# OpenBMB/VisRAG

Measured on AMD Instinct MI355X. Metric: page-images embedded/sec (VisRAG-Ret encode, 448x448, bf16 MFMA) + queries/sec@top-10 over 100k-page index, higher is better.
Workload: dtype bf16; 1 GPU; VisRAG-Ret (SigLIP-so400m 26 blk + resampler + MiniCPM-2B 40 layers) bf16 encode batch=32 page images 448x448 per GPU; index 100000 rows x 2304 sharded 1 way(s), 1000 queries top-10; batch_per_gpu=32, global_batch=32, parallelism=dp1 (pages sharded, no data-path collective)

## Files before the change

visrag_amd/csrc/gemm256w.hip:

```cpp
#include <type_traits>

#include "gemm_core.h"
#include "gemm_epilogue.h"
#include "gemm256w_acc.h"

namespace vr {

bool gemm256w_fits(const GemmArgs& a, int bn);

namespace {

constexpr int W_STAGE = 2 * G256_TILE_BYTES;
constexpr unsigned W_OOB = 0x80000000u;

}

constexpr int W_STAGING = 4096;
constexpr int W_WARM_DUMP = 256;
constexpr int W_SMEM_BYTES = 2 * W_STAGE + 4 * W_STAGING + 4 * W_WARM_DUMP;

constexpr bool warm_shares_tile(size_t bytes, unsigned total) {
    unsigned at = 0;
    for (unsigned w = 0; w < total; ++w)
        for (unsigned v = 0; v < WARM_WAVES; ++v) {
            const WarmShare s = warm_share(bytes, w, total, v);
            if (s.first != at || s.end < s.first) return false;
            at = s.end;
        }
    return at == warm_lines(bytes) && (size_t)at * WARM_LINE >= bytes && (bytes == 0 || (size_t)(at - 1) * WARM_LINE < bytes);
}
static_assert(warm_shares_tile(0, 1) && warm_shares_tile(0, 243), "no lines");
static_assert(warm_shares_tile(1, 1) && warm_shares_tile(WARM_LINE, 4) && warm_shares_tile(WARM_LINE + 1, 4), "1 and 2 lines");
static_assert(warm_shares_tile(63 * WARM_LINE, 1) && warm_shares_tile(64 * WARM_LINE, 1) && warm_shares_tile(65 * WARM_LINE, 1), "63 / 64 / 65 lines, one workgroup");
static_assert(warm_shares_tile(63 * WARM_LINE, 4) && warm_shares_tile(64 * WARM_LINE, 4) && warm_shares_tile(65 * WARM_LINE - 3, 4), "63 / 64 / 65 lines, four");
static_assert(warm_shares_tile(100 * WARM_LINE, 243) && warm_shares_tile(5 * WARM_LINE, 405), "a region of fewer lines than the grid has waves");
static_assert(warm_shares_tile((size_t)2304 * 2304 * 2, 243), "W_o (10.6 MB) over the decoder's q|k|v grid");
static_assert(warm_shares_tile((size_t)2304 * 5760 * 2, 405), "W_down (26.5 MB) over the decoder's gate|up grid");
static_assert(warm_shares_tile(WARM_MAX_BYTES - 1, 1021), "the largest region");
static_assert(warm_cut((1u << 24) - 1, 65534, 65535) == (unsigned)(((1ull << 24) - 1) * 65534 / 65535) && warm_cut(65534, 65534, 65535) == 65533 &&
              warm_cut((1u << 24) - 1, 65535, 65535) == (1u << 24) - 1, "the largest grid of the 32-bit form");
static_assert(warm_part(0, warm_lines(WARM_MAX_BYTES - 1), 65536, 65537).end == warm_lines(WARM_MAX_BYTES - 1) &&
              warm_cut(1u << 24, 70001, 70003) == (unsigned)((1ull << 24) * 70001 / 70003) && warm_cut(82944, 100, 243) == 82944ull * 100 / 243, "both forms of the cut");
#if VR_WARM_LINE == 128
static_assert(warm_instructions(warm_share((size_t)2304 * 2304 * 2, 0, 243, 0)) == 2 &&
              warm_instructions(warm_share((size_t)2304 * 5760 * 2, 404, 405, 3)) == 2, "two requests per wave in the decoder");
#endif

#define W_KERNEL_TEMPLATE template <int EPI, bool PLAIN, int NJ>
#define W_KERNEL_NAME gemm256w_bf16_kernel
#include "gemm256w_kernel.h"
#undef W_KERNEL_TEMPLATE
#undef W_KERNEL_NAME

template <int EPI, bool PLAIN, int NJ>
static hipError_t launch_wp(GemmArgs a, hipStream_t s) {
    constexpr int BN = 32 * NJ;
    const int tn = (a.N + BN - 1) / BN, tm = (a.M + G256_BM - 1) / G256_BM;
    if (a.raster_gm <= 0) a.raster_gm = tm <= 16 ? tm : 4;
    if (!gemm256w_fits(a, BN)) return hipErrorInvalidValue;
    if (gemm_args_refused(a, EPI, NJ == 6 ? GEMM_VARIANT_192W : GEMM_VARIANT_256W)) return hipErrorInvalidValue;
    int total = tn * tm;
    if (a.ksplit > 1) total *= a.ksplit;
    auto k = gemm256w_bf16_kernel<EPI, PLAIN, NJ>;
    static unsigned long long attr = 0;
    set_max_dynamic_lds((const void*)k, W_SMEM_BYTES, attr);
    hipLaunchKernelGGL(k, dim3(total), dim3(256), W_SMEM_BYTES, s, a);
    return hipGetLastError();
}

template <int EPI>
static hipError_t launch_w(const GemmArgs& a, hipStream_t s) {
    if constexpr (EPI == EPI_BF16 || EPI == EPI_GELU || EPI == EPI_SWIGLU || EPI == EPI_ROPE) {
        const bool rb_ok = !a.rowbias || (EPI == EPI_BF16 && a.rowbias_period > 0 && a.rowbias_period % G256_BM == 0 && a.rowbias_cols % 64 == 0 && a.rowbias_cols <= a.rowbias_ld &&
                                          (size_t)a.rowbias_period * a.rowbias_ld * 4 < (1ull << 32));
        if (!a.rowmap && rb_ok && (a.N & 7) == 0 && (a.ldo & 7) == 0) return launch_wp<EPI, true, 8>(a, s);
    }
    return launch_wp<EPI, false, 8>(a, s);
}

bool gemm256w_fits(const GemmArgs& a, int bn) {
    const size_t tm = (a.M + G256_BM - 1) / G256_BM, tn = (a.N + bn - 1) / bn;
    return tm * G256_BM * (size_t)a.lda * 2 < (1ull << 31) && tn * bn * (size_t)a.ldw * 2 < (1ull << 31) &&
           (size_t)G256_BM * (size_t)a.ldo * 4 < (1ull << 31) && (!a.rowbias || (size_t)G256_BM * (size_t)a.rowbias_ld * 4 < (1ull << 31));
}

hipError_t launch_gemm256w(const GemmArgs& a, int epi, hipStream_t s) {
    switch (epi) {
        case EPI_BF16: return launch_w<EPI_BF16>(a, s);
        case EPI_GELU: return launch_w<EPI_GELU>(a, s);
        case EPI_F32: return launch_w<EPI_F32>(a, s);
        case EPI_RESID: return launch_w<EPI_RESID>(a, s);
        case EPI_SWIGLU: return launch_w<EPI_SWIGLU>(a, s);
        case EPI_ROPE: return launch_w<EPI_ROPE>(a, s);
        default: return hipErrorInvalidValue;
    }
}

hipError_t launch_gemm192w(const GemmArgs& a, int epi, hipStream_t s) {
    if (a.N % 192) return hipErrorInvalidValue;
    if (epi == EPI_RESID && a.ksplit <= 1) return launch_wp<EPI_RESID, false, 6>(a, s);
    if (epi == EPI_F32) return launch_wp<EPI_F32, false, 6>(a, s);
    return hipErrorInvalidValue;
}

}
```

visrag_amd/csrc/gemm256w_kernel.h:

```cpp
W_KERNEL_TEMPLATE
__global__ __launch_bounds__(256) __attribute__((amdgpu_waves_per_eu(1, 1))) void W_KERNEL_NAME(GemmArgs p) {
    static_assert(NJ == 8 || (NJ == 6 && !PLAIN), "wave tile 128 x 128 or 128 x 96");
    constexpr int BN = 32 * NJ;
    constexpr int NS = 8 * NJ;
    constexpr int NR = 8 + NJ;
    constexpr int DS = NJ == 8 ? 5 : 4;
    constexpr int SB1 = NS * 5 / 8;
    constexpr int D1 = (NS - 1 - (SB1 + 2)) / DS + 1;
    constexpr int SB2 = NJ;
    constexpr int NF = NJ / 2;
    static_assert(SB2 + 3 + DS * (NR - D1 - 1) < NS && SB2 + 2 + 2 * (NR - 1) < NS && 2 * NR - 2 < SB1, "schedule fits");
    extern __shared__ __attribute__((aligned(16))) char smem[];
#ifdef VR_W_TIMING
    const unsigned long long tm0 = __builtin_amdgcn_s_memrealtime();
    unsigned long long tm1 = 0, tm2 = 0, cy1 = 0, cy2 = 0;
#endif
    const int tiles_n = (p.N + BN - 1) / BN;
    const int tiles_m = (p.M + G256_BM - 1) / G256_BM;
    const int ks = p.ksplit > 1 ? p.ksplit : 1;
    const int total = tiles_m * tiles_n * ks;
    const int Ks = p.K / ks;
    const int nk = Ks / GEMM_BK;

    const int my_first = xcd_remap(blockIdx.x, total);
// ... 31 lines not shown

    typedef const __attribute__((address_space(3))) bf16x8* frag_p;
    frag_p pA[2][2], pW[2][2];
#pragma unroll
    for (int st = 0; st < 2; ++st)
#pragma unroll
        for (int kk = 0; kk < 2; ++kk) {
            const int ch = ((kk * 4 + fq) ^ (fr & 7)) << 4;
            pA[st][kk] = (frag_p)VR_LDS(smem + st * W_STAGE + (wm * 128 + fr) * 128 + ch);
            pW[st][kk] = (frag_p)VR_LDS(smem + st * W_STAGE + G256_TILE_BYTES + (wn * 16 * NJ + fr) * 128 + ch);
            asm volatile("" : "+v"(pA[st][kk]), "+v"(pW[st][kk]));
        }

    bf16x8 a0[8], w0[NJ], a1[8], w1[NJ];
    int m0, n0, split;
    coords(my_first, m0, n0, split);
    unsigned curA = tile_off_a(m0, split), curW = tile_off_w(n0, split);
    unsigned warm_lo = 0, warm_hi = 0;

    {
        const unsigned k1 = nk > 1 ? (unsigned)(GEMM_BK * 2) : W_OOB;
#pragma unroll
        for (int d = 0; d < NR; ++d) dma(0, d, lofA + curA, lofW + curW);
#pragma unroll
        for (int d = 0; d < NR; ++d) dma(1, d, lofA + curA + k1, lofW + curW + k1);
        if constexpr (NJ == 8) {
            if (p.warm && p.warm_bytes) {
                const WarmShare sh = warm_share(p.warm_bytes, (unsigned)my_first, (unsigned)total, (unsigned)wave);
                warm_lo = (unsigned)__builtin_amdgcn_readfirstlane((int)sh.first);
                warm_hi = (unsigned)__builtin_amdgcn_readfirstlane((int)sh.end);
            }
        }
        W_FOR_EACH_ACC(W_ZERO)
        if constexpr (NJ == 8) VR_WAIT_VM_BARRIER(16); else VR_WAIT_VM_BARRIER(14);
#pragma unroll
        for (int j = 0; j < NJ; ++j) w0[j] = pW[0][0][j * 128];
#pragma unroll
        for (int i = 0; i < 8; ++i) a0[i] = pA[0][0][i * 128];
    }
#ifdef VR_W_TIMING
    asm volatile("s_waitcnt lgkmcnt(0)" ::: "memory");
    tm1 = __builtin_amdgcn_s_memrealtime();
    cy1 = __builtin_amdgcn_s_memtime();
#endif

    {
        const unsigned nxtA = W_OOB, nxtW = W_OOB;

        auto step = [&](auto stage_c, int kt) {
            constexpr int S = decltype(stage_c)::value;
            const int k2 = kt + 2;
            const unsigned vA = lofA + (k2 < nk ? curA + (unsigned)k2 * (GEMM_BK * 2) : nxtA + (unsigned)(k2 - nk) * (GEMM_BK * 2));
            const unsigned vW = lofW + (k2 < nk ? curW + (unsigned)k2 * (GEMM_BK * 2) : nxtW + (unsigned)(k2 - nk) * (GEMM_BK * 2));
            __builtin_amdgcn_sched_barrier(0);
            auto aux1 = [&](int sl) {
                if (sl < 2 * NR && (sl & 1) == 0) {
                    const int q = sl >> 1;
                    if (q < NJ) w1[q] = pW[S][1][q * 128];
                    else a1[q - NJ] = pA[S][1][(q - NJ) * 128];
                }
                if (sl == SB1) asm volatile("s_waitcnt lgkmcnt(0)\n\ts_barrier" ::: "memory");
                if (sl >= SB1 + 2 && (sl - (SB1 + 2)) % DS == 0) dma(S, (sl - (SB1 + 2)) / DS, vA, vW);
                __builtin_amdgcn_sched_barrier(0);
            };
            auto aux2 = [&](int sl) {
                if (sl == SB2) { if constexpr (D1 == 5) VR_WAIT_VM_BARRIER(5); else VR_WAIT_VM_BARRIER(4); }
                if (sl >= SB2 + 3 && (sl - (SB2 + 3)) % DS == 0 && D1 + (sl - (SB2 + 3)) / DS < NR)
                    dma(S, D1 + (sl - (SB2 + 3)) / DS, vA, vW);
                if (sl >= SB2 + 2 && sl < SB2 + 2 + 2 * NR && ((sl - SB2) & 1) == 0) {
                    const int q = (sl - (SB2 + 2)) >> 1;
                    if (q < NJ) w0[q] = pW[S ^ 1][0][q * 128];
                    else a0[q - NJ] = pA[S ^ 1][0][(q - NJ) * 128];
                }
                __builtin_amdgcn_sched_barrier(0);
            };
#define W_P1(n, R, C0, C1, C2, C3) \
            if (((n) & 7) < NJ) { W_MFMA(R, C0, C1, C2, C3, w0[(n) & 7], a0[(n) >> 3]); aux1(((n) >> 3) * NJ + ((n) & 7)); }
#define W_P2(n, R, C0, C1, C2, C3) \
            if (((n) & 7) < NJ) { W_MFMA(R, C0, C1, C2, C3, w1[(n) & 7], a1[(n) >> 3]); aux2(((n) >> 3) * NJ + ((n) & 7)); }
            W_FOR_EACH_ACC(W_P1)
            W_FOR_EACH_ACC(W_P2)
#undef W_P1
#undef W_P2
        };

        for (int kt = 0; kt < nk; kt += 2) {
            step(std::integral_constant<int, 0>{}, kt);
            if (kt + 1 >= nk) break;
            step(std::integral_constant<int, 1>{}, kt + 1);
        }
        asm volatile("s_nop 15\n\ts_nop 15" ::: "memory");
#ifdef VR_W_TIMING
        tm2 = __builtin_amdgcn_s_memrealtime();
        cy2 = __builtin_amdgcn_s_memtime();
#endif

        const int mrow0 = m0 + wm * 128, nb0 = n0 + wn * (16 * NJ);
        char* const wl0 = smem + 2 * W_STAGE + wave * W_STAGING;
        bool plain_resid = false;
        if constexpr (EPI == EPI_RESID) plain_resid = !p.rowmap;
        auto uni32 = [](unsigned v) { return (unsigned)__builtin_amdgcn_readfirstlane((int)v); };
        auto uni_ptr = [&](const void* q) {
            const unsigned long long a = (unsigned long long)q;
            return (void*)(((unsigned long long)uni32((unsigned)(a >> 32)) << 32) | uni32((unsigned)a));
        };
        auto warm_requests = [&]() {
            if constexpr (NJ == 8) {
                if (warm_lo < warm_hi) {
                    const unsigned long long wa = (unsigned long long)uni_ptr(p.warm);
                    const auto wrs = __builtin_amdgcn_make_buffer_rsrc((void*)wa, 0, uni32((unsigned)p.warm_bytes), 0x00020000);
                    const unsigned pad = (0u - (unsigned)wa) & 3u;
                    char* const dump = smem + 2 * W_STAGE + 4 * W_STAGING + wave * W_WARM_DUMP;
                    auto request = [&](unsigned l) {
                        const unsigned line = l + (unsigned)lane;
                        __builtin_amdgcn_raw_ptr_buffer_load_lds(wrs, VR_LDS(dump), 4, line < warm_hi ? line * WARM_LINE + pad : W_OOB, 0, 0, 0);
                    };
                    __builtin_amdgcn_sched_barrier(0);
                    request(warm_lo);
                    request(warm_lo + 64);
                    __builtin_amdgcn_sched_barrier(0);
#pragma nounroll
                    for (unsigned l = warm_lo + 128; l < warm_hi; l += 64) request(l);
                }
            }
        };
        bool buf_tile = false;
        if constexpr (EPI == EPI_RESID) buf_tile = plain_resid && n0 + BN <= p.N;
        if constexpr (EPI == EPI_F32) buf_tile = !p.rowmap && !p.rowbias && n0 + BN <= p.N;
        if constexpr (EPI == EPI_RESID || EPI == EPI_F32) {
            if (buf_tile) {
                constexpr int MI = 2;
                const float alpha = __builtin_bit_cast(float, uni32(__builtin_bit_cast(unsigned, p.alpha)));
                const unsigned ldb = uni32((unsigned)p.ldo * 4u);
                const unsigned nrec = uni32((unsigned)min(G256_BM, p.M - m0) * ldb);
                float* obase = (float*)p.out + (size_t)m0 * p.ldo;
                if constexpr (EPI == EPI_F32) obase += (size_t)split * p.split_stride;
                const auto ors = __builtin_amdgcn_make_buffer_rsrc(uni_ptr(obase), 0, nrec, 0x00020000);
                const bool with_bias = p.bias && (EPI == EPI_RESID || split == 0);
                const auto brs = __builtin_amdgcn_make_buffer_rsrc(uni_ptr(p.bias), 0, uni32(with_bias ? (unsigned)p.N * 4u : 0u), 0x00020000);
                const unsigned voff = (unsigned)(wm * 128 + fr) * ldb + (unsigned)(nb0 + fq * 4) * 4u;
                f32x4 bias[NJ];
#pragma unroll
                for (int j = 0; j < NJ; ++j)
                    bias[j] = __builtin_bit_cast(f32x4, __builtin_amdgcn_raw_buffer_load_b128(brs, (unsigned)(nb0 + fq * 4) * 4u + j * 64, 0, 0));
                if constexpr (EPI == EPI_RESID) {
                    constexpr int RD = NJ == 6 ? 3 : 2;
                    const auto rrs = __builtin_amdgcn_make_buffer_rsrc(uni_ptr(p.resid + (size_t)m0 * p.ldo), 0, nrec, 0x00020000);
                    f32x4 rs[RD + 1][MI][NF];
                    auto load_piece = [&](int q, f32x4 (&dst)[MI][NF]) {
                        const int h = q & 1, sg = q >> 1;
#pragma unroll
                        for (int i = 0; i < MI; ++i)
#pragma unroll
                            for (int j = 0; j < NF; ++j)
                                dst[i][j] = __builtin_bit_cast(f32x4, __builtin_amdgcn_raw_buffer_load_b128(
                                    rrs, voff + (unsigned)((sg * MI + i) * 16) * ldb + (h * NF + j) * 64, 0, 0));
                    };
#pragma unroll
                    for (int q = 0; q < RD; ++q) load_piece(q, rs[q]);
                    warm_requests();
#pragma unroll
                    for (int q = 0; q < 8; ++q) {
                        const int h = q & 1, sg = q >> 1;
                        if (q + RD < 8) load_piece(q + RD, rs[(q + RD) % (RD + 1)]);
                        f32x4 acc[MI][NF];
#define W_RD(n, R, C0, C1, C2, C3) \
                        if (((n) & 7) < NJ && ((n) & 7) / NF == h && ((n) >> 4) == sg) W_READ(acc[((n) >> 3) & 1][((n) & 7) % NF], C0, C1, C2, C3);
                        W_FOR_EACH_ACC(W_RD)
#undef W_RD
#pragma unroll
                        for (int i = 0; i < MI; ++i)
#pragma unroll
                            for (int j = 0; j < NF; ++j) {
                                const f32x4 v = rs[q % (RD + 1)][i][j] + alpha * (acc[i][j] + bias[h * NF + j]);
                                __builtin_amdgcn_raw_buffer_store_b128(__builtin_bit_cast(u32x4, v), ors,
                                                                       voff + (unsigned)((sg * MI + i) * 16) * ldb + (h * NF + j) * 64, 0, 0);
                            }
                        __builtin_amdgcn_sched_barrier(0);
                    }
                } else {
                    warm_requests();
#pragma unroll
                    for (int q = 0; q < 8; ++q) {
                        const int h = q & 1, sg = q >> 1;
                        f32x4 acc[MI][NF];
#define W_RD(n, R, C0, C1, C2, C3) \
                        if (((n) & 7) < NJ && ((n) & 7) / NF == h && ((n) >> 4) == sg) W_READ(acc[((n) >> 3) & 1][((n) & 7) % NF], C0, C1, C2, C3);
                        W_FOR_EACH_ACC(W_RD)
#undef W_RD
#pragma unroll
                        for (int i = 0; i < MI; ++i)
#pragma unroll
                            for (int j = 0; j < NF; ++j)
                                __builtin_amdgcn_raw_buffer_store_b128(__builtin_bit_cast(u32x4, acc[i][j] + bias[h * NF + j]), ors,
                                                                       voff + (unsigned)((sg * MI + i) * 16) * ldb + (h * NF + j) * 64, 0, 0);
                        __builtin_amdgcn_sched_barrier(0);
                    }
                }
            }
        }
        if constexpr (EPI == EPI_RESID) {
            if (plain_resid && !buf_tile) {
                constexpr int MI = 2;
                const float* __restrict__ resid = p.resid;
                float* __restrict__ out = (float*)p.out;
                constexpr int RD = 1;
                f32x4 rs[RD + 1][MI][NF];
                auto load_piece = [&](int q, f32x4 (&dst)[MI][NF]) {
                    const int h = q & 1, sg = q >> 1;
#pragma unroll
                    for (int i = 0; i < MI; ++i) {
                        const size_t ro = (size_t)min(mrow0 + (sg * MI + i) * 16 + fr, p.M - 1) * p.ldo;
#pragma unroll
                        for (int j = 0; j < NF; ++j) {
                            dst[i][j] = *reinterpret_cast<const f32x4*>(resid + ro + min(nb0 + (h * NF + j) * 16 + fq * 4, p.N - 4));
                        }
                    }
                };
#pragma unroll
                for (int q = 0; q < RD; ++q) load_piece(q, rs[q]);
                f32x4 bias[NJ];
#pragma unroll
                for (int j = 0; j < NJ; ++j)
                    bias[j] = p.bias ? *reinterpret_cast<const f32x4*>(p.bias + min(nb0 + j * 16 + fq * 4, p.N - 4)) : f32x4{0.f, 0.f, 0.f, 0.f};
                warm_requests();
#pragma unroll
                for (int q = 0; q < 8; ++q) {
                    const int h = q & 1, sg = q >> 1;
                    if (q + RD < 8) load_piece(q + RD, rs[(q + RD) % (RD + 1)]);
                    f32x4 acc[MI][NF];
#define W_RD(n, R, C0, C1, C2, C3) \
                    if (((n) & 7) < NJ && ((n) & 7) / NF == h && ((n) >> 4) == sg) W_READ(acc[((n) >> 3) & 1][((n) & 7) % NF], C0, C1, C2, C3);
                    W_FOR_EACH_ACC(W_RD)
#undef W_RD
#pragma unroll
                    for (int i = 0; i < MI; ++i) {
                        const int m = mrow0 + (sg * MI + i) * 16 + fr;
#pragma unroll
                        for (int j = 0; j < NF; ++j) {
                            const int n = nb0 + (h * NF + j) * 16 + fq * 4;
                            if (m < p.M && n < p.N)
                                *reinterpret_cast<f32x4*>(out + (size_t)m * p.ldo + n) = rs[q % (RD + 1)][i][j] + p.alpha * (acc[i][j] + bias[h * NF + j]);
                        }
                    }
                    __builtin_amdgcn_sched_barrier(0);
                }
            }
        }
        if (!plain_resid && !buf_tile) {
            const unsigned ldo2 = uni32((unsigned)p.ldo * 2u);
            const auto ors16 = __builtin_amdgcn_make_buffer_rsrc(uni_ptr((const char*)p.out + (size_t)m0 * p.ldo * 2), 0,
                                                                 uni32((unsigned)min(G256_BM, p.M - m0) * ldo2), 0x00020000);
            f32x4 biasw[NJ];
            if constexpr (PLAIN && NF == 4 && EPI != EPI_ROPE) {
                const auto brs = __builtin_amdgcn_make_buffer_rsrc(uni_ptr(p.bias), 0, uni32(p.bias ? (unsigned)p.N * 4u : 0u), 0x00020000);
#pragma unroll
                for (int j = 0; j < NJ; ++j)
                    biasw[j] = __builtin_bit_cast(f32x4, __builtin_amdgcn_raw_buffer_load_b128(brs, (unsigned)(nb0 + fq * 4) * 4u + j * 64, 0, 0));
            }
            const bool rb_on = EPI == EPI_BF16 && PLAIN && p.rowbias != nullptr;
            const auto rbrs = __builtin_amdgcn_make_buffer_rsrc(uni_ptr(p.rowbias), 0,
                                                                uni32(rb_on ? (unsigned)p.rowbias_period * (unsigned)p.rowbias_ld * 4u : 0u), 0x00020000);
            const unsigned rb_row0 = rb_on ? uni32((unsigned)(m0 % p.rowbias_period)) : 0u;
            int posw[8];
#pragma unroll
            for (int t = 0; t < 8; ++t) posw[t] = 0;
            if constexpr (EPI == EPI_ROPE && PLAIN) {
#pragma unroll
                for (int t = 0; t < 8; ++t) posw[t] = p.rope_pos[min(mrow0 + t * 16 + fr, p.M - 1)];
            }
            f32x4 rt[2][2][4];
            auto load_rope = [&](int sg, f32x4 (&d)[2][4]) {
#pragma unroll
                for (int i = 0; i < 2; ++i) {
                    const float* tab = p.rope_table + (size_t)posw[sg * 2 + i] * 64 + fq * 4;
#pragma unroll
                    for (int j = 0; j < 4; ++j) d[i][j] = *reinterpret_cast<const f32x4*>(tab + j * 16);
                }
            };
            if constexpr (EPI == EPI_ROPE && PLAIN) load_rope(0, rt[0]);
            (void)ors16; (void)ldo2; (void)biasw; (void)rbrs; (void)rb_row0; (void)posw; (void)rt;
            warm_requests();
#pragma unroll
            for (int q = 0; q < 8; ++q) {
                constexpr int MI = 2;
                const int h = q & 1, sg = q >> 1;
                f32x4 acc[MI][NF];
#define W_RD(n, R, C0, C1, C2, C3) \
                if (((n) & 7) < NJ && ((n) & 7) / NF == h && ((n) >> 4) == sg) W_READ(acc[((n) >> 3) & 1][((n) & 7) % NF], C0, C1, C2, C3);
                W_FOR_EACH_ACC(W_RD)
#undef W_RD
                const int mr = mrow0 + sg * 32, nb = nb0 + h * (16 * NF);
                bool done = false;
                if constexpr (EPI == EPI_F32) {
                    if (!p.rowmap && !p.rowbias) {
                        float* __restrict__ out = (float*)p.out + (size_t)split * p.split_stride;
                        const float* bp = split == 0 ? p.bias : nullptr;
                        f32x4 bias[NF];
#pragma unroll
                        for (int j = 0; j < NF; ++j)
                            bias[j] = bp ? *reinterpret_cast<const f32x4*>(bp + min(nb + j * 16 + fq * 4, p.N - 4)) : f32x4{0.f, 0.f, 0.f, 0.f};
#pragma unroll
                        for (int i = 0; i < MI; ++i) {
                            const int m = mr + i * 16 + fr;
#pragma unroll
                            for (int j = 0; j < NF; ++j) {
                                const int n = nb + j * 16 + fq * 4;
                                if (m < p.M && n < p.N) *reinterpret_cast<f32x4*>(out + (size_t)m * p.ldo + n) = acc[i][j] + bias[j];
                            }
                        }
                        done = true;
                    } else if (ks > 1) {
                        GemmArgs ps = p;
                        ps.out = (float*)p.out + (size_t)split * p.split_stride;
                        if (split > 0) ps.bias = nullptr;
#pragma unroll
                        for (int i = 0; i < MI; ++i) gemm_epilogue_row<EPI_F32, NF>(acc[i], ps, mr + i * 16 + fr, nb, fq);
                        done = true;
                    }
                }
                if constexpr (EPI == EPI_RESID) {
#pragma unroll
                    for (int i = 0; i < MI; ++i) gemm_epilogue_row<EPI_RESID, NF>(acc[i], p, mr + i * 16 + fr, nb, fq);
                    done = true;
                }
                if constexpr (NF == 4 && (EPI == EPI_BF16 || EPI == EPI_GELU || EPI == EPI_SWIGLU || EPI == EPI_ROPE)) {
                    if constexpr (PLAIN) {
                        f32x4 b4[4];
#pragma unroll
                        for (int j = 0; j < 4; ++j) b4[j] = EPI == EPI_ROPE ? f32x4{0.f, 0.f, 0.f, 0.f} : biasw[h * NF + j];
                        if constexpr (EPI == EPI_ROPE) { if (h == 0 && sg + 1 < 4) load_rope(sg + 1, rt[(sg + 1) & 1]); }
                        gemm_epilogue_tile_lds_plain_buf<EPI, MI>(acc, b4, p, ors16, (unsigned)(wm * 128 + sg * 32) * ldo2, ldo2, rt[sg & 1], nb, lane, wl0,
                                                                  rbrs, (rb_row0 + (unsigned)(wm * 128 + sg * 32)) * (unsigned)p.rowbias_ld * 4u);
                        done = true;
                    } else if ((p.N & 7) == 0 && (p.ldo & 7) == 0) {
                        gemm_epilogue_tile_lds<EPI, MI>(acc, p, mr, nb, lane, wl0);
                        done = true;
                    }
                }
                if constexpr (!PLAIN) {
                    if (!done) {
#pragma unroll
                        for (int i = 0; i < MI; ++i) gemm_epilogue_row<EPI, NF>(acc[i], p, mr + i * 16 + fr, nb, fq);
                    }
                }
                if (!PLAIN || (q & 1)) __builtin_amdgcn_sched_barrier(0);
            }
        }
    }
#ifdef VR_W_TIMING
    if (threadIdx.x == 0 && p.rope_table) {
        const unsigned long long tm3 = __builtin_amdgcn_s_memrealtime();
        asm volatile("s_waitcnt vmcnt(0)" ::: "memory");
        const unsigned long long tm4 = __builtin_amdgcn_s_memrealtime();
        unsigned long long* d = (unsigned long long*)p.rope_table + (size_t)blockIdx.x * 16;
        d[0] = tm0; d[1] = tm1; d[2] = tm2; d[3] = tm3; d[4] = tm4;
        d[5] = __builtin_amdgcn_s_getreg((31 << 11) | 4);
        d[6] = __builtin_amdgcn_s_getreg((31 << 11) | 20);
        d[7] = cy2 - cy1;
    }
#endif
}
```

visrag_amd/csrc/gemm_epilogue.h:

```cpp
#pragma once
#include "common.h"
#include "kernels.h"

namespace vr {

__device__ __forceinline__ float gelu_erf(float x) {
    constexpr float X0 = 4.2426406871192851f;
    const float xc = fminf(fmaxf(x, -X0), X0);
    const float u = xc * xc;
    float p = 1.125353832e-10f;
    p = fmaf(p, u, -1.074373991e-08f);
    p = fmaf(p, u, 4.536592962e-07f);
    p = fmaf(p, u, -1.129243078e-05f);
    p = fmaf(p, u, 1.871812565e-04f);
    p = fmaf(p, u, -2.218800626e-03f);
    p = fmaf(p, u, 1.963623831e-02f);
    p = fmaf(p, u, -1.326938473e-01f);
    p = fmaf(p, u, 7.978062550e-01f);
    const float e = xc * p;
    const float hx = 0.5f * x;
    return fmaf(hx, e, hx);
}
__device__ __forceinline__ f32x4 gelu_erf4(f32x4 x) {
    constexpr float X0 = 4.2426406871192851f;
// ... 196 lines not shown
    if constexpr (EPI == EPI_SWIGLU) {
#pragma unroll
        for (int it = 0; it < MI; ++it) {
            const int row = it * 16 + (lane >> 2), c = lane & 3;
            const u32x4 d = *reinterpret_cast<const u32x4*>(wl + row * 128 + ((c ^ (row & 3)) << 4));
            const int m = mrow0 + row, n = nb / 2 + c * 8;
            if (m < p.M && 2 * n < p.N) {
                const int orow = p.rowmap ? p.rowmap[m] : m;
                if (orow >= 0) *reinterpret_cast<u32x4*>(out + (size_t)orow * p.ldo + n) = d;
            }
        }
    } else {
#pragma unroll
        for (int it = 0; it < MI * 2; ++it) {
            const int row = it * 8 + (lane >> 3), c = lane & 7;
            const u32x4 d = *reinterpret_cast<const u32x4*>(wl + row * 128 + ((c ^ (row & 7)) << 4));
            const int m = mrow0 + row, n = nb + c * 8;
            if (m < p.M && n < p.N) {
                const int orow = p.rowmap ? p.rowmap[m] : m;
                if (orow >= 0) *reinterpret_cast<u32x4*>(out + (size_t)orow * p.ldo + n) = d;
            }
        }
    }
}

template <int EPI, int MI>
__device__ __forceinline__ void gemm_epilogue_tile_lds_plain(f32x4 (&acc)[MI][4], const GemmArgs& p, int mrow0, int nb,
                                                             int lane, char* wl_generic) {
    typedef __attribute__((address_space(3))) char* lds_p;
    const lds_p wl = (lds_p)VR_LDS(wl_generic);
    const int fr = lane & 15, fq = lane >> 4;
    if constexpr (EPI == EPI_SWIGLU) {
        f32x4 bias[4];
#pragma unroll
        for (int j = 0; j < 4; ++j) bias[j] = f32x4{0.f, 0.f, 0.f, 0.f};
        if (p.bias) {
#pragma unroll
            for (int j = 0; j < 4; ++j) bias[j] = *reinterpret_cast<const f32x4*>(p.bias + min(nb + j * 16 + fq * 4, p.N - 4));
        }
#pragma unroll
        for (int i = 0; i < MI; ++i) {
            const int row = i * 16 + fr;
#pragma unroll
            for (int jj = 0; jj < 2; ++jj) {
                const f32x4 g = acc[i][2 * jj] + bias[2 * jj], u = acc[i][2 * jj + 1] + bias[2 * jj + 1];
                bf16x4 o;
#pragma unroll
                for (int r = 0; r < 4; ++r) o[r] = f2bf(silu(g[r]) * u[r]);
                const int c = jj * 2 + (fq >> 1);
                *reinterpret_cast<__attribute__((address_space(3))) bf16x4*>(wl + row * 128 + ((c ^ (row & 3)) << 4) + (fq & 1) * 8) = o;
            }
        }
    } else {
        f32x4 bias[4];
#pragma unroll
        for (int j = 0; j < 4; ++j) bias[j] = f32x4{0.f, 0.f, 0.f, 0.f};
        if constexpr (EPI == EPI_BF16 || EPI == EPI_GELU) {
            if (p.bias) {
#pragma unroll
                for (int j = 0; j < 4; ++j) bias[j] = *reinterpret_cast<const f32x4*>(p.bias + min(nb + j * 16 + fq * 4, p.N - 4));
            }
        }
        if constexpr (EPI == EPI_ROPE) {
            if (nb < p.rope_cols && nb < p.N) {
                int pos[MI];
#pragma unroll
                for (int i = 0; i < MI; ++i) pos[i] = p.rope_pos[min(mrow0 + i * 16 + fr, p.M - 1)];
#pragma unroll
                for (int c = 0; c < MI; c += 2) {
                    f32x4 cs[2][2], sn[2][2];
#pragma unroll
                    for (int ii = 0; ii < 2; ++ii) {
                        const float* tab = p.rope_table + (size_t)pos[c + ii] * 64;
#pragma unroll
                        for (int j = 0; j < 2; ++j) {
                            cs[ii][j] = *reinterpret_cast<const f32x4*>(tab + j * 16 + fq * 4);
                            sn[ii][j] = *reinterpret_cast<const f32x4*>(tab + 32 + j * 16 + fq * 4);
                        }
                    }
#pragma unroll
                    for (int ii = 0; ii < 2; ++ii)
#pragma unroll
                        for (int j = 0; j < 2; ++j) {
                            const f32x4 x1 = acc[c + ii][j], x2 = acc[c + ii][j + 2];
                            acc[c + ii][j] = x1 * cs[ii][j] - x2 * sn[ii][j];
                            acc[c + ii][j + 2] = x2 * cs[ii][j] + x1 * sn[ii][j];
                        }
                }
            }
        }
        if constexpr (EPI == EPI_BF16) {
            if (nb < p.col_scale_n) {
#pragma unroll
                for (int j = 0; j < 4; ++j) {
                    bias[j] *= p.col_scale;
#pragma unroll
                    for (int i = 0; i < MI; ++i) acc[i][j] *= p.col_scale;
                }
            }
        }
#pragma unroll
        for (int i = 0; i < MI; ++i) {
            const int row = i * 16 + fr;
#pragma unroll
            for (int j = 0; j < 4; ++j) {
                f32x4 v = acc[i][j] + bias[j];
                if constexpr (EPI == EPI_GELU) v = gelu_erf4(v);
                const bf16x4 o = __builtin_convertvector(v, bf16x4);
                const int c = j * 2 + (fq >> 1);
                *reinterpret_cast<__attribute__((address_space(3))) bf16x4*>(wl + row * 128 + ((c ^ (row & 7)) << 4) + (fq & 1) * 8) = o;
            }
        }
    }
    bf16_t* out = (bf16_t*)p.out;
    if constexpr (EPI == EPI_SWIGLU) {
        u32x4 d[MI];
#pragma unroll
        for (int it = 0; it < MI; ++it) {
            const int row = it * 16 + (lane >> 2), c = lane & 3;
            d[it] = *reinterpret_cast<const __attribute__((address_space(3))) u32x4*>(wl + row * 128 + ((c ^ (row & 3)) << 4));
        }
#pragma unroll
        for (int it = 0; it < MI; ++it) {
            const int row = it * 16 + (lane >> 2), c = lane & 3;
            const int m = mrow0 + row, n = nb / 2 + c * 8;
            if (m < p.M && 2 * n < p.N) *reinterpret_cast<u32x4*>(out + (size_t)m * p.ldo + n) = d[it];
        }
    } else {
        u32x4 d[MI * 2];
#pragma unroll
        for (int it = 0; it < MI * 2; ++it) {
            const int row = it * 8 + (lane >> 3), c = lane & 7;
            d[it] = *reinterpret_cast<const __attribute__((address_space(3))) u32x4*>(wl + row * 128 + ((c ^ (row & 7)) << 4));
        }
#pragma unroll
        for (int it = 0; it < MI * 2; ++it) {
            const int row = it * 8 + (lane >> 3), c = lane & 7;
            const int m = mrow0 + row, n = nb + c * 8;
            if (m < p.M && n < p.N) *reinterpret_cast<u32x4*>(out + (size_t)m * p.ldo + n) = d[it];
        }
    }
}

template <int EPI, int MI>
__device__ __forceinline__ void gemm_epilogue_tile_lds_plain_buf(f32x4 (&acc)[MI][4], f32x4 (&bias)[4], const GemmArgs& p,
                                                                 __amdgpu_buffer_rsrc_t ors, unsigned row_off, unsigned ldo_bytes,
                                                                 const f32x4 (&rope)[MI][4], int nb, int lane, char* wl_generic,
                                                                 __amdgpu_buffer_rsrc_t rbrs, unsigned rb_off) {
    static_assert(EPI == EPI_BF16 || EPI == EPI_GELU || EPI == EPI_SWIGLU || EPI == EPI_ROPE, "bf16 outputs only");
    typedef __attribute__((address_space(3))) char* lds_p;
    const lds_p wl = (lds_p)VR_LDS(wl_generic);
    const int fr = lane & 15, fq = lane >> 4;
    if constexpr (EPI == EPI_SWIGLU) {
#pragma unroll
        for (int i = 0; i < MI; ++i) {
            const int row = i * 16 + fr;
#pragma unroll
            for (int jj = 0; jj < 2; ++jj) {
                const f32x4 g = acc[i][2 * jj] + bias[2 * jj], u = acc[i][2 * jj + 1] + bias[2 * jj + 1];
                bf16x4 o;
#pragma unroll
                for (int r = 0; r < 4; ++r) o[r] = f2bf(silu(g[r]) * u[r]);
                const int c = jj * 2 + (fq >> 1);
                *reinterpret_cast<__attribute__((address_space(3))) bf16x4*>(wl + row * 128 + ((c ^ (row & 3)) << 4) + (fq & 1) * 8) = o;
            }
        }
    } else {
        if constexpr (EPI == EPI_ROPE) {
            if (nb < p.rope_cols && nb < p.N) {
#pragma unroll
                for (int i = 0; i < MI; ++i)
#pragma unroll
                    for (int j = 0; j < 2; ++j) {
                        const f32x4 x1 = acc[i][j], x2 = acc[i][j + 2];
                        acc[i][j] = x1 * rope[i][j] - x2 * rope[i][2 + j];
                        acc[i][j + 2] = x2 * rope[i][j] + x1 * rope[i][2 + j];
                    }
            }
        }
        if constexpr (EPI == EPI_BF16) {
            if (p.rowbias && nb < p.rowbias_cols) {
                f32x4 rb[MI][4];
#pragma unroll
                for (int i = 0; i < MI; ++i)
#pragma unroll
                    for (int j = 0; j < 4; ++j)
                        rb[i][j] = __builtin_bit_cast(f32x4, __builtin_amdgcn_raw_buffer_load_b128(
                            rbrs, rb_off + (unsigned)(i * 16 + fr) * (unsigned)p.rowbias_ld * 4u + (unsigned)(nb + j * 16 + fq * 4) * 4u, 0, 0));
#pragma unroll
                for (int i = 0; i < MI; ++i)
#pragma unroll
                    for (int j = 0; j < 4; ++j) acc[i][j] += rb[i][j];
            }
            if (nb < p.col_scale_n) {
#pragma unroll
                for (int j = 0; j < 4; ++j) {
#pragma unroll
                    for (int i = 0; i < MI; ++i) acc[i][j] = (acc[i][j] + bias[j]) * p.col_scale;
                }
            } else {
#pragma unroll
                for (int j = 0; j < 4; ++j)
#pragma unroll
                    for (int i = 0; i < MI; ++i) acc[i][j] += bias[j];
            }
        }
#pragma unroll
        for (int i = 0; i < MI; ++i) {
            const int row = i * 16 + fr;
#pragma unroll
            for (int j = 0; j < 4; ++j) {
                f32x4 v = acc[i][j];
                if constexpr (EPI == EPI_GELU) v = gelu_erf4(v + bias[j]);
                const bf16x4 o = __builtin_convertvector(v, bf16x4);
                const int c = j * 2 + (fq >> 1);
                *reinterpret_cast<__attribute__((address_space(3))) bf16x4*>(wl + row * 128 + ((c ^ (row & 7)) << 4) + (fq & 1) * 8) = o;
            }
        }
    }
    constexpr unsigned OOR = 0x80000000u;
    if constexpr (EPI == EPI_SWIGLU) {
        u32x4 d[MI];
#pragma unroll
        for (int it = 0; it < MI; ++it) {
            const int row = it * 16 + (lane >> 2), c = lane & 3;
            d[it] = *reinterpret_cast<const __attribute__((address_space(3))) u32x4*>(wl + row * 128 + ((c ^ (row & 3)) << 4));
        }
        const int n = nb / 2 + (lane & 3) * 8;
        const unsigned cofs = 2 * n < p.N ? (unsigned)n * 2u : OOR;
#pragma unroll
        for (int it = 0; it < MI; ++it)
            __builtin_amdgcn_raw_buffer_store_b128(d[it], ors, row_off + (unsigned)(it * 16 + (lane >> 2)) * ldo_bytes + cofs, 0, 0);
    } else {
        u32x4 d[MI * 2];
#pragma unroll
        for (int it = 0; it < MI * 2; ++it) {
            const int row = it * 8 + (lane >> 3), c = lane & 7;
            d[it] = *reinterpret_cast<const __attribute__((address_space(3))) u32x4*>(wl + row * 128 + ((c ^ (row & 7)) << 4));
        }
        const int n = nb + (lane & 7) * 8;
        const unsigned cofs = n < p.N ? (unsigned)n * 2u : OOR;
#pragma unroll
        for (int it = 0; it < MI * 2; ++it)
            __builtin_amdgcn_raw_buffer_store_b128(d[it], ors, row_off + (unsigned)(it * 8 + (lane >> 3)) * ldo_bytes + cofs, 0, 0);
    }
}

template <int EPI, int MI>
__device__ __forceinline__ void gemm_epilogue_tile_lds(f32x4 (&acc)[MI][4], const GemmArgs& p, int mrow0, int nb,
                                                       int lane, char* wl) {
    if (!p.rowmap && !p.rowbias) gemm_epilogue_tile_lds_plain<EPI, MI>(acc, p, mrow0, nb, lane, wl);
    else gemm_epilogue_tile_lds_general<EPI, MI>(acc, p, mrow0, nb, lane, wl);
}

}
```

visrag_amd/csrc/ops.hip:

```cpp
#include <hip/hip_runtime.h>

#include <algorithm>
#include <chrono>
#include <map>
#include <tuple>
#include <vector>

#include "engine_common.h"

struct ResizeTab { DevBuf bounds, kk; int ksize = 0; };
static std::map<std::tuple<int, int, int>, ResizeTab> g_resize_tabs;

static int get_resize_tab(int dev, int in_size, int out_size, ResizeTab** out) {
    auto key = std::make_tuple(dev, in_size, out_size);
    auto it = g_resize_tabs.find(key);
    if (it == g_resize_tabs.end()) {
        std::vector<int> b, k;
        ResizeTab t;
        t.ksize = resize_coeffs(in_size, out_size, b, k);
        VRCHK(t.bounds.alloc(b.size() * 4));
        VRCHK(t.kk.alloc(k.size() * 4));
        HIPCHK(hipMemcpy(t.bounds.p, b.data(), b.size() * 4, hipMemcpyHostToDevice));
        HIPCHK(hipMemcpy(t.kk.p, k.data(), k.size() * 4, hipMemcpyHostToDevice));
        it = g_resize_tabs.emplace(key, std::move(t)).first;
    }
    *out = &it->second;
    return VR_OK;
}

struct ResizeScratch { DevBuf in, tmp; };
static std::map<std::pair<int, void*>, ResizeScratch> g_resize_scratch;

extern "C" int vr_resize_bicubic(int device_id, const uint8_t* src, int32_t src_on_device, int32_t H, int32_t W,
                                 uint8_t* dst, int32_t out_h, int32_t out_w, void* stream) {
    if (!src || !dst || H <= 0 || W <= 0 || out_h <= 0 || out_w <= 0) return fail(VR_ERR_INVALID, "bad resize arguments");
    VRCHK(set_dev(device_id));
    hipStream_t s = (hipStream_t)stream;
    ResizeScratch& sc = g_resize_scratch[std::make_pair(device_id, stream)];
    const uint8_t* in = src;
    if (!src_on_device) {
        VRCHK(sc.in.reserve((size_t)H * W * 3));
        HIPCHK(hipMemcpyAsync(sc.in.p, src, (size_t)H * W * 3, hipMemcpyHostToDevice, s));
        in = sc.in.as<uint8_t>();
    }
    const bool need_h = out_w != W, need_v = out_h != H;
    if (!need_h && !need_v) {
        HIPCHK(hipMemcpyAsync(dst, in, (size_t)H * W * 3, hipMemcpyDeviceToDevice, s));
    } else {
        const uint8_t* mid = in;
        if (need_h) {
            ResizeTab* th = nullptr;
            VRCHK(get_resize_tab(device_id, W, out_w, &th));
            uint8_t* hout = dst;
            if (need_v) { VRCHK(sc.tmp.reserve((size_t)H * out_w * 3)); hout = sc.tmp.as<uint8_t>(); }
            HIPCHK(launch_resize_h(in, W, H, hout, out_w, th->bounds.as<int>(), th->kk.as<int>(), th->ksize, s));
            mid = hout;
        }
        if (need_v) {
            ResizeTab* tv = nullptr;
            VRCHK(get_resize_tab(device_id, H, out_h, &tv));
            HIPCHK(launch_resize_v(mid, out_w, dst, out_h, tv->bounds.as<int>(), tv->kk.as<int>(), tv->ksize, s));
        }
    }
    if (!src_on_device) HIPCHK(hipStreamSynchronize(s));
    return VR_OK;
}

extern "C" int vr_synth_pages(int device_id, uint8_t* out, int32_t n, int32_t size, int64_t seed, int64_t first, void* stream) {
    if (!out || n < 0 || size < 64 || size > 4096) return fail(VR_ERR_INVALID, "bad synth_pages arguments");
    VRCHK(set_dev(device_id));
    HIPCHK(launch_synth_pages(out, n, size, seed, first, (hipStream_t)stream));
    return VR_OK;
}

__global__ void spin_kernel(long long ticks) {
    const long long t0 = wall_clock64();
    while (wall_clock64() - t0 < ticks) __builtin_amdgcn_s_sleep(8);
}

extern "C" int vr_streams_overlap(int device_id, void* stream_a, void* stream_b, int32_t* overlap) {
    if (!overlap) return fail(VR_ERR_INVALID, "NULL argument");
    VRCHK(set_dev(device_id));
    const hipStream_t a = (hipStream_t)stream_a, b = (hipStream_t)stream_b;
    constexpr int usec = 400;
    int votes = 0;
    for (int rep = 0; rep < 3; ++rep) {
        HIPCHK(hipStreamSynchronize(a));
        HIPCHK(hipStreamSynchronize(b));
        const auto t0 = std::chrono::steady_clock::now();
        hipLaunchKernelGGL(spin_kernel, dim3(1), dim3(1), 0, a, (long long)usec * 100);
        hipLaunchKernelGGL(spin_kernel, dim3(1), dim3(1), 0, b, (long long)usec * 100);
        HIPCHK(hipGetLastError());
        HIPCHK(hipStreamSynchronize(a));
        HIPCHK(hipStreamSynchronize(b));
        const double us = std::chrono::duration<double, std::micro>(std::chrono::steady_clock::now() - t0).count();
        if (rep > 0) votes += us < 1.6 * usec ? 1 : 0;
    }
    *overlap = votes == 2 ? 1 : 0;
    return VR_OK;
}

extern "C" int vr_op_gemm_warm(int device_id, const void* A, int32_t lda, const void* W, int32_t ldw, int32_t M, int32_t N,
                               int32_t K, int32_t epilogue, const float* bias, const float* resid, float alpha, void* out,
                               int32_t ldo, const int32_t* rope_pos, const float* rope_table, int32_t rope_cols,
                               int32_t variant, const vr_gemm_extras_t* extras, const void* warm, uint64_t warm_bytes, void* stream) {
    if (!A || !W || !out) return fail(VR_ERR_INVALID, "NULL argument");
    if (variant != GEMM_VARIANT_GLDS && variant != GEMM_VARIANT_AUTO && variant != GEMM_VARIANT_192 && variant != GEMM_VARIANT_256IL && variant != GEMM_VARIANT_256W && variant != GEMM_VARIANT_192W &&
        variant != GEMM_VARIANT_128W_192 && variant != GEMM_VARIANT_128W_256)
        return fail(VR_ERR_INVALID, "variant %d: 0 (128^2 tile), 3 (auto), 7 (256x192 tile), 9 (256^2 tile), 12 / 13 (256^2 / 256x192 tile, one wave per SIMD), 14 / 15 (128x192 / 128x256 tile, one wave per SIMD)", variant);
    if (((variant == 7 || variant == 13 || variant == 14) ? N % 192 : N % 128) || K % 64 || M <= 0) return fail(VR_ERR_INVALID, "need N %% 128 == 0 (192 for variant 7), K %% 64 == 0");
    if (epilogue == EPI_RESID && !resid) return fail(VR_ERR_INVALID, "EPI_RESID needs resid");
    if (epilogue == EPI_ROPE && (!rope_pos || !rope_table)) return fail(VR_ERR_INVALID, "EPI_ROPE needs tables");
    VRCHK(set_dev(device_id));
    GemmArgs a{};
    a.A = A; a.lda = lda; a.W = W; a.ldw = ldw; a.M = M; a.N = N; a.K = K; a.bias = bias; a.resid = resid;
    a.alpha = alpha; a.out = out; a.ldo = ldo; a.rope_pos = rope_pos; a.rope_table = rope_table; a.rope_cols = rope_cols;
    if (extras) {
        a.rowmap = extras->rowmap;
        a.rowbias = extras->rowbias; a.rowbias_period = extras->rowbias_period; a.rowbias_ld = extras->rowbias_ld; a.rowbias_cols = extras->rowbias_cols;
        a.col_scale = extras->col_scale; a.col_scale_n = extras->col_scale_n;
        a.ksplit = extras->ksplit; a.split_stride = (size_t)extras->split_stride;
        a.m_dev = extras->m_dev; a.m_sub = extras->m_sub;
        a.raster_gm = extras->raster_gm;
    }
    a.warm = warm; a.warm_bytes = (size_t)warm_bytes;
    HIPCHK(launch_gemm(a, epilogue, variant, (hipStream_t)stream));
    return VR_OK;
}

extern "C" int vr_op_gemm_ex(int device_id, const void* A, int32_t lda, const void* W, int32_t ldw, int32_t M, int32_t N,
                             int32_t K, int32_t epilogue, const float* bias, const float* resid, float alpha, void* out,
                             int32_t ldo, const int32_t* rope_pos, const float* rope_table, int32_t rope_cols,
                             int32_t variant, const vr_gemm_extras_t* extras, void* stream) {
    return vr_op_gemm_warm(device_id, A, lda, W, ldw, M, N, K, epilogue, bias, resid, alpha, out, ldo, rope_pos, rope_table, rope_cols,
                           variant, extras, nullptr, 0, stream);
}

extern "C" int vr_op_gemm(int device_id, const void* A, int32_t lda, const void* W, int32_t ldw, int32_t M, int32_t N,
                          int32_t K, int32_t epilogue, const float* bias, const float* resid, float alpha, void* out,
                          int32_t ldo, const int32_t* rope_pos, const float* rope_table, int32_t rope_cols,
                          int32_t variant, void* stream) {
    return vr_op_gemm_ex(device_id, A, lda, W, ldw, M, N, K, epilogue, bias, resid, alpha, out, ldo, rope_pos, rope_table, rope_cols,
                         variant, nullptr, stream);
}

extern "C" int vr_op_norm(int device_id, int32_t kind, const float* x, int32_t rows, int32_t dim, const float* weight,
                          const float* bias, float eps, void* out, int32_t ldo, void* stream) {
    if (!x || !weight || !out || (kind == 0 && !bias)) return fail(VR_ERR_INVALID, "NULL argument");
    VRCHK(set_dev(device_id));
    if (kind == 0) HIPCHK(launch_layernorm(x, rows, dim, dim, weight, bias, eps, out, ldo, (hipStream_t)stream));
    else HIPCHK(launch_rmsnorm(x, rows, dim, dim, weight, eps, out, ldo, (hipStream_t)stream));
    return VR_OK;
}

extern "C" int vr_op_attention_ex(int device_id, const void* q, int32_t ldq, const void* k, int32_t ldk, const void* v,
                                  int32_t ldv, void* out, int32_t ldo, const int32_t* cu_q, const int32_t* cu_kv, int32_t B,
                                  int32_t heads, int32_t head_dim, int32_t max_q, int32_t causal, int32_t q_shared,
                                  float scale, const vr_attn_extras_t* extras, void* stream) {
    if (!q || !k || !v || !out || !cu_q || !cu_kv) return fail(VR_ERR_INVALID, "NULL argument");
    VRCHK(set_dev(device_id));
    AttnArgs a{};
    a.q = q; a.ldq = ldq; a.k = k; a.ldk = ldk; a.v = v; a.ldv = ldv; a.out = out; a.ldo = ldo; a.cu_q = cu_q;
    a.cu_kv = cu_kv; a.B = B; a.heads = heads; a.head_dim = head_dim; a.max_q = max_q; a.causal = causal;
    a.q_shared = q_shared; a.scale = scale;
    if (extras) {
        a.kv_group = extras->kv_group; a.kv_end = extras->kv_end; a.q_in_rows = extras->q_in_rows;
        a.q_head_stride = extras->q_head_stride; a.q_prescaled = extras->q_prescaled; a.lse = extras->lse;
    }
    HIPCHK(launch_attention(a, (hipStream_t)stream));
    return VR_OK;
}

extern "C" int vr_op_attention(int device_id, const void* q, int32_t ldq, const void* k, int32_t ldk, const void* v,
                               int32_t ldv, void* out, int32_t ldo, const int32_t* cu_q, const int32_t* cu_kv, int32_t B,
                               int32_t heads, int32_t head_dim, int32_t max_q, int32_t causal, int32_t q_shared,
                               float scale, void* stream) {
    return vr_op_attention_ex(device_id, q, ldq, k, ldk, v, ldv, out, ldo, cu_q, cu_kv, B, heads, head_dim, max_q, causal, q_shared,
                              scale, nullptr, stream);
}

extern "C" int vr_op_attn_combine(int device_id, const void* part, const float* lse, int32_t S, const int32_t* S_dev, int32_t heads,
                                  int32_t group, int32_t n_rows, void* out, int32_t ld_out, const void* W, int32_t ldw, int32_t M,
                                  int32_t N, int32_t K, int32_t ksplit, int32_t planes, int32_t ldo, int64_t split_stride, void* stream) {
    if (!part || !lse || !out) return fail(VR_ERR_INVALID, "NULL argument");
    if (heads < 1 || n_rows < 1 || n_rows > 16) return fail(VR_ERR_INVALID, "need heads >= 1 and 1..16 rows");
    if (!S_dev && (S < 1 || S > GEN_ATT_SPLITS)) return fail(VR_ERR_INVALID, "S must be 1..%d", GEN_ATT_SPLITS);
    VRCHK(set_dev(device_id));
    if (!W) {
        if (ld_out < heads * 128 && n_rows > 1) return fail(VR_ERR_INVALID, "ld_out must cover heads * 128");
        HIPCHK(launch_attn_combine(part, lse, S, heads, group, out, (hipStream_t)stream, S_dev, n_rows, ld_out));
        return VR_OK;
    }
    if (n_rows != 1) return fail(VR_ERR_INVALID, "the fused form merges one row");
    if (N < 1 || N % 4 || K < 64 || K % 64 || ldw < K || ldw % 8) return fail(VR_ERR_INVALID, "need N %% 4 == 0, K %% 64 == 0, ldw >= K, ldw %% 8 == 0");
    if (ksplit < 1 || ksplit > planes) return fail(VR_ERR_INVALID, "ksplit must be 1..planes");
    if (ldo < N || ldo % 4 || (ksplit > 1 && (split_stride < (int64_t)(M > 0 ? M : 1) * ldo || split_stride % 4)))
        return fail(VR_ERR_INVALID, "ldo must cover N, split_stride a plane of M x ldo; both multiples of 4");
    if (((uintptr_t)W | (uintptr_t)out) & 15) return fail(VR_ERR_INVALID, "pointers must be 16-byte aligned");
    GemmArgs a{};
    a.A = nullptr; a.lda = K; a.W = W; a.ldw = ldw; a.M = M; a.N = N; a.K = K; a.out = out; a.ldo = ldo;
    a.ksplit = ksplit; a.split_stride = (size_t)split_stride;
    const SkinnyCombine cb{part, lse, S, heads, group, S_dev};
    HIPCHK(launch_gemm_skinny(a, (hipStream_t)stream, false, &cb));
    return VR_OK;
}

extern "C" int vr_op_gemm_skinny(int device_id, const void* A, int32_t lda, const void* W, int32_t ldw, int32_t M, int32_t N,
                                 int32_t K, int32_t ksplit, const float* bias, int32_t swiglu, void* out, int32_t ldo,
                                 int64_t split_stride, void* stream) {
    if (!A || !W || !out) return fail(VR_ERR_INVALID, "NULL argument");
    if (M < 1 || N < 1 || K < 64 || K % 64 || N % 4) return fail(VR_ERR_INVALID, "need M >= 1, N %% 4 == 0, K %% 64 == 0");
    if (M > 32 || (swiglu && M > 16)) return fail(VR_ERR_CAPACITY, "%d rows: at most 32 (16 with swiglu)", M);
    if (ksplit < 1 || ksplit > 64) return fail(VR_ERR_INVALID, "ksplit must be 1..64");
    if (lda < K || ldw < K || lda % 8 || ldw % 8) return fail(VR_ERR_INVALID, "lda / ldw must cover K and be multiples of 8");
    if (((uintptr_t)A | (uintptr_t)W | (uintptr_t)out | (uintptr_t)bias) & 15) return fail(VR_ERR_INVALID, "pointers must be 16-byte aligned");
    if (swiglu) {
        if (ksplit != 1 || N % 32) return fail(VR_ERR_INVALID, "swiglu needs ksplit 1 and N %% 32 == 0");
        if (ldo < N / 2 || ldo % 8) return fail(VR_ERR_INVALID, "swiglu: ldo must cover N / 2 and be a multiple of 8");
    } else {
        if (ldo < N || ldo % 4) return fail(VR_ERR_INVALID, "ldo must cover N and be a multiple of 4");
        if (ksplit > 1 && (split_stride < (int64_t)M * ldo || split_stride % 4)) return fail(VR_ERR_INVALID, "split_stride must cover a plane of M x ldo and be a multiple of 4");
    }
    VRCHK(set_dev(device_id));
    GemmArgs a{};
    a.A = A; a.lda = lda; a.W = W; a.ldw = ldw; a.M = M; a.N = N; a.K = K; a.bias = bias; a.out = out; a.ldo = ldo;
    a.ksplit = ksplit; a.split_stride = (size_t)split_stride;
    HIPCHK(launch_gemm_skinny(a, (hipStream_t)stream, swiglu != 0));
    return VR_OK;
}

extern "C" int vr_op_plane_sum(int device_id, int32_t kind, const float* parts, int32_t nsplit, int64_t split_stride, int32_t ldp,
                               int32_t rows, int32_t dim, float* x, int32_t ldx, float alpha, const float* weight, float eps,
                               void* out, int32_t ldo, void* stream) {
    if (!parts) return fail(VR_ERR_INVALID, "NULL argument");
    if (kind != 0 && kind != 1) return fail(VR_ERR_INVALID, "kind %d: 0 (residual + RMSNorm), 1 (SwiGLU)", kind);
    if (rows < 1 || dim < 1 || nsplit < 1 || nsplit > 64) return fail(VR_ERR_INVALID, "need rows, dim >= 1 and nsplit 1..64");
    if (split_stride % 4 || (nsplit > 1 && split_stride < (int64_t)rows * ldp)) return fail(VR_ERR_INVALID, "split_stride must cover a plane of rows x ldp and be a multiple of 4");
    VRCHK(set_dev(device_id));
    if (kind == 0) {
        if (!x || (out && !weight)) return fail(VR_ERR_INVALID, "NULL argument");
        if (dim > 3584 || (out && ldo > 3584)) return fail(VR_ERR_CAPACITY, "rows of at most 3584 columns");
        if (dim % 4 || ldx % 4 || ldp % 4 || ldx < dim || ldp < dim || (out && (ldo % 4 || ldo < dim)))
            return fail(VR_ERR_INVALID, "dim, ldx, ldp, ldo must be multiples of 4 and the strides cover dim");
        if (((uintptr_t)parts | (uintptr_t)x | (uintptr_t)weight) & 15 || (uintptr_t)out & 7) return fail(VR_ERR_INVALID, "misaligned pointer");
        HIPCHK(launch_rmsnorm_accum(x, rows, dim, ldx, parts, nsplit, (size_t)split_stride, ldp, alpha, weight, eps, out, ldo, (hipStream_t)stream));
    } else {
        if (!out) return fail(VR_ERR_INVALID, "NULL argument");
        if (dim % 16 || ldp < 2 * dim || ldo < dim) return fail(VR_ERR_INVALID, "swiglu: dim %% 16 == 0, ldp >= 2 dim, ldo >= dim");
        HIPCHK(launch_swiglu_sum(parts, nsplit, (size_t)split_stride, ldp, rows, dim, out, ldo, (hipStream_t)stream));
    }
    return VR_OK;
}

static std::map<int, DevBuf> g_chat_op_scratch;

extern "C" int vr_op_chat_attention(int device_id, const void* q, const void* prompt, const void* tails, int32_t layers, int32_t l,
                                    int32_t E, int32_t slots, int32_t max_len, int32_t rows, int32_t max_new, int32_t n,
                                    const int32_t* step_row, const int32_t* step_slot, const int32_t* step_tail,
                                    const int32_t* slot_plen, int32_t force_splits, void* att, void* stream) {
    if (!q || !prompt || !tails || !step_row || !step_slot || !step_tail || !slot_plen || !att) return fail(VR_ERR_INVALID, "NULL argument");
    if (E < 64 || E % 64) return fail(VR_ERR_INVALID, "E must be a multiple of the head dim 64");
    if (layers < 1 || l < 0 || l >= layers) return fail(VR_ERR_INVALID, "layer %d of %d", l, layers);
    if (slots < 1 || max_len < 1 || rows < 1 || max_new < 1) return fail(VR_ERR_INVALID, "bad cache geometry");
// ... 313 lines not shown
```

Baseline: 710.4 pages/s.

## Store SwiGLU epilogue via permlane16 swap, bypassing LDS; relax 192w N checks

The SwiGLU epilogue no longer stages the bf16 results through LDS. Lanes exchange halves with permlane16_swap and each lane writes a 16-byte buffer store directly, which removes an LDS write/read round trip and its bank traffic from the epilogue. The 192w/256w variants now accept N that is a multiple of 64 for the residual epilogue, relying on out-of-range buffer stores. The change also adds timing-only switches that skip parts of the residual epilogue, which are compiled in only when a timing macro is defined.

After: 708.4 pages/s. No clear change (-0.3%).

```diff
diff --git a/visrag_amd/csrc/gemm256w.hip b/visrag_amd/csrc/gemm256w.hip
--- a/visrag_amd/csrc/gemm256w.hip
+++ b/visrag_amd/csrc/gemm256w.hip
@@ -44,6 +44,12 @@
 #if VR_WARM_LINE == 128
 static_assert(warm_instructions(warm_share((size_t)2304 * 2304 * 2, 0, 243, 0)) == 2 &&
               warm_instructions(warm_share((size_t)2304 * 5760 * 2, 404, 405, 3)) == 2, "two requests per wave in the decoder");
+#endif
+
+#if defined(VR_W_TIMING) && defined(VR_W_EPI_SKIP)
+constexpr int W_EPI_SKIP = VR_W_EPI_SKIP;
+#else
+constexpr int W_EPI_SKIP = 0;
 #endif
 
 #define W_KERNEL_TEMPLATE template <int EPI, bool PLAIN, int NJ>
@@ -97,7 +103,7 @@
 }
 
 hipError_t launch_gemm192w(const GemmArgs& a, int epi, hipStream_t s) {
-    if (a.N % 192) return hipErrorInvalidValue;
+    if (a.N % 192 && (a.N % 64 || epi != EPI_RESID || a.ksplit > 1)) return hipErrorInvalidValue;
     if (epi == EPI_RESID && a.ksplit <= 1) return launch_wp<EPI_RESID, false, 6>(a, s);
     if (epi == EPI_F32) return launch_wp<EPI_F32, false, 6>(a, s);
     return hipErrorInvalidValue;
diff --git a/visrag_amd/csrc/gemm256w_kernel.h b/visrag_amd/csrc/gemm256w_kernel.h
--- a/visrag_amd/csrc/gemm256w_kernel.h
+++ b/visrag_amd/csrc/gemm256w_kernel.h
@@ -207,9 +207,11 @@
 #pragma unroll
                         for (int i = 0; i < MI; ++i)
 #pragma unroll
-                            for (int j = 0; j < NF; ++j)
-                                dst[i][j] = __builtin_bit_cast(f32x4, __builtin_amdgcn_raw_buffer_load_b128(
+                            for (int j = 0; j < NF; ++j) {
+                                if constexpr (W_EPI_SKIP & 4) dst[i][j] = bias[j];
+                                else dst[i][j] = __builtin_bit_cast(f32x4, __builtin_amdgcn_raw_buffer_load_b128(
                                     rrs, voff + (unsigned)((sg * MI + i) * 16) * ldb + (h * NF + j) * 64, 0, 0));
+                            }
                     };
 #pragma unroll
                     for (int q = 0; q < RD; ++q) load_piece(q, rs[q]);
@@ -227,9 +229,12 @@
                         for (int i = 0; i < MI; ++i)
 #pragma unroll
                             for (int j = 0; j < NF; ++j) {
-                                const f32x4 v = rs[q % (RD + 1)][i][j] + alpha * (acc[i][j] + bias[h * NF + j]);
-                                __builtin_amdgcn_raw_buffer_store_b128(__builtin_bit_cast(u32x4, v), ors,
-                                                                       voff + (unsigned)((sg * MI + i) * 16) * ldb + (h * NF + j) * 64, 0, 0);
+                                f32x4 v = rs[q % (RD + 1)][i][j];
+                                if constexpr (W_EPI_SKIP & 2) v = __builtin_bit_cast(f32x4, __builtin_bit_cast(u32x4, v) | __builtin_bit_cast(u32x4, acc[i][j]));
+                                else v += alpha * (acc[i][j] + bias[h * NF + j]);
+                                if constexpr (W_EPI_SKIP & 1) asm volatile("" : : "v"(v));
+                                else __builtin_amdgcn_raw_buffer_store_b128(__builtin_bit_cast(u32x4, v), ors,
+                                                                            voff + (unsigned)((sg * MI + i) * 16) * ldb + (h * NF + j) * 64, 0, 0);
                             }
                         __builtin_amdgcn_sched_barrier(0);
                     }
@@ -404,11 +409,12 @@
         }
     }
 #ifdef VR_W_TIMING
-    if (threadIdx.x == 0 && p.rope_table) {
+    const void* const rec = EPI == EPI_ROPE ? (const void*)p.resid : (const void*)p.rope_table;
+    if (threadIdx.x == 0 && rec) {
         const unsigned long long tm3 = __builtin_amdgcn_s_memrealtime();
         asm volatile("s_waitcnt vmcnt(0)" ::: "memory");
         const unsigned long long tm4 = __builtin_amdgcn_s_memrealtime();
-        unsigned long long* d = (unsigned long long*)p.rope_table + (size_t)blockIdx.x * 16;
+        unsigned long long* d = (unsigned long long*)rec + (size_t)blockIdx.x * 16;
         d[0] = tm0; d[1] = tm1; d[2] = tm2; d[3] = tm3; d[4] = tm4;
         d[5] = __builtin_amdgcn_s_getreg((31 << 11) | 4);
         d[6] = __builtin_amdgcn_s_getreg((31 << 11) | 20);
diff --git a/visrag_amd/csrc/gemm_epilogue.h b/visrag_amd/csrc/gemm_epilogue.h
--- a/visrag_amd/csrc/gemm_epilogue.h
+++ b/visrag_amd/csrc/gemm_epilogue.h
@@ -372,19 +372,24 @@
     const lds_p wl = (lds_p)VR_LDS(wl_generic);
     const int fr = lane & 15, fq = lane >> 4;
     if constexpr (EPI == EPI_SWIGLU) {
+        constexpr unsigned OOR = 0x80000000u;
+        const int n = nb / 2 + (fq & 1) * 16 + (fq & 2) * 4;
+        const unsigned cofs = 2 * n < p.N ? (unsigned)n * 2u : OOR;
 #pragma unroll
         for (int i = 0; i < MI; ++i) {
-            const int row = i * 16 + fr;
+            bf16x4 o[2];
 #pragma unroll
             for (int jj = 0; jj < 2; ++jj) {
                 const f32x4 g = acc[i][2 * jj] + bias[2 * jj], u = acc[i][2 * jj + 1] + bias[2 * jj + 1];
-                bf16x4 o;
-#pragma unroll
-                for (int r = 0; r < 4; ++r) o[r] = f2bf(silu(g[r]) * u[r]);
-                const int c = jj * 2 + (fq >> 1);
-                *reinterpret_cast<__attribute__((address_space(3))) bf16x4*>(wl + row * 128 + ((c ^ (row & 3)) << 4) + (fq & 1) * 8) = o;
-            }
-        }
+#pragma unroll
+                for (int r = 0; r < 4; ++r) o[jj][r] = f2bf(silu(g[r]) * u[r]);
+            }
+            const u32x2 x = __builtin_bit_cast(u32x2, o[0]), y = __builtin_bit_cast(u32x2, o[1]);
+            const u32x2 lo = __builtin_amdgcn_permlane16_swap(x[0], y[0], false, false);
+            const u32x2 hi = __builtin_amdgcn_permlane16_swap(x[1], y[1], false, false);
+            __builtin_amdgcn_raw_buffer_store_b128(u32x4{lo[0], hi[0], lo[1], hi[1]}, ors, row_off + (unsigned)(i * 16 + fr) * ldo_bytes + cofs, 0, 0);
+        }
+        (void)wl;
     } else {
         if constexpr (EPI == EPI_ROPE) {
             if (nb < p.rope_cols && nb < p.N) {
@@ -439,19 +444,7 @@
         }
     }
     constexpr unsigned OOR = 0x80000000u;
-    if constexpr (EPI == EPI_SWIGLU) {
-        u32x4 d[MI];
-#pragma unroll
-        for (int it = 0; it < MI; ++it) {
-            const int row = it * 16 + (lane >> 2), c = lane & 3;
-            d[it] = *reinterpret_cast<const __attribute__((address_space(3))) u32x4*>(wl + row * 128 + ((c ^ (row & 3)) << 4));
-        }
-        const int n = nb / 2 + (lane & 3) * 8;
-        const unsigned cofs = 2 * n < p.N ? (unsigned)n * 2u : OOR;
-#pragma unroll
-        for (int it = 0; it < MI; ++it)
-            __builtin_amdgcn_raw_buffer_store_b128(d[it], ors, row_off + (unsigned)(it * 16 + (lane >> 2)) * ldo_bytes + cofs, 0, 0);
-    } else {
+    if constexpr (EPI != EPI_SWIGLU) {
         u32x4 d[MI * 2];
 #pragma unroll
         for (int it = 0; it < MI * 2; ++it) {
diff --git a/visrag_amd/csrc/ops.hip b/visrag_amd/csrc/ops.hip
--- a/visrag_amd/csrc/ops.hip
+++ b/visrag_amd/csrc/ops.hip
@@ -108,7 +108,8 @@
     if (variant != GEMM_VARIANT_GLDS && variant != GEMM_VARIANT_AUTO && variant != GEMM_VARIANT_192 && variant != GEMM_VARIANT_256IL && variant != GEMM_VARIANT_256W && variant != GEMM_VARIANT_192W &&
         variant != GEMM_VARIANT_128W_192 && variant != GEMM_VARIANT_128W_256)
         return fail(VR_ERR_INVALID, "variant %d: 0 (128^2 tile), 3 (auto), 7 (256x192 tile), 9 (256^2 tile), 12 / 13 (256^2 / 256x192 tile, one wave per SIMD), 14 / 15 (128x192 / 128x256 tile, one wave per SIMD)", variant);
-    if (((variant == 7 || variant == 13 || variant == 14) ? N % 192 : N % 128) || K % 64 || M <= 0) return fail(VR_ERR_INVALID, "need N %% 128 == 0 (192 for variant 7), K %% 64 == 0");
+    const int n_mult = (variant == GEMM_VARIANT_256W || variant == GEMM_VARIANT_192W) ? 64 : (variant == 7 || variant == 14) ? 192 : 128;
+    if (N % n_mult || K % 64 || M <= 0) return fail(VR_ERR_INVALID, "need N %% 128 == 0 (192 for variants 7 and 14, 64 for 12 and 13), K %% 64 == 0");
     if (epilogue == EPI_RESID && !resid) return fail(VR_ERR_INVALID, "EPI_RESID needs resid");
     if (epilogue == EPI_ROPE && (!rope_pos || !rope_table)) return fail(VR_ERR_INVALID, "EPI_ROPE needs tables");
     VRCHK(set_dev(device_id));
```
